# praveenpenumaka/splat-transform

Measured on AMD Instinct MI355X. Metric: Msplats/sec PLY->SOG (SH-3, 10 k-means iters), higher is better.
Workload: dtype f64+f32 (bit-exact JS semantics); fp16 MFMA (f32 accumulate) for the assign prefilter

## Files before the change

### splat-transform_amd/csrc/st_kmeans_nd.hip

```cpp
#include <cmath>
#include <cstring>
#include <utility>

#include "st_kmeans.h"

namespace st {
namespace {

using namespace km;

template <typename F, int... I>
__device__ inline void static_for_(F &f, std::integer_sequence<int, I...>) {
    (f(std::integral_constant<int, I>{}), ...);
}
template <int N, typename F>
__device__ inline void static_for(F &&f) {
    static_for_(f, std::make_integer_sequence<int, N>{});
}

typedef _Float16 f16x8 __attribute__((ext_vector_type(8)));
typedef float f32x16 __attribute__((ext_vector_type(16)));
typedef float f32x2 __attribute__((ext_vector_type(2)));

constexpr int PT = 4;
constexpr int NW = 4;
constexpr int WG = 64 * NW;
constexpr int CT_STAGE = 8;
enum { UPD_ALWAYS = 0, UPD_LANE = 1, UPD_WAVE = 2, UPD_BOTH = 3, UPD_DEFAULT = UPD_BOTH };
constexpr int CAND_CAP = 64;
constexpr int CAND_CAP2 = 2048;
constexpr int OVF_BATCH = 4096;
uint32_t sumnd_big() {
    const char *e = getenv("ST_SUMND_BIG");
    return e ? (uint32_t)std::max(1ul, strtoul(e, nullptr, 10)) : 16384u;
}

int sweep_update() {
    const char *e = getenv("ST_SWEEP_UPDATE");
    if (!e || !*e) return UPD_DEFAULT;
    if (!strcmp(e, "always")) return UPD_ALWAYS;
    if (!strcmp(e, "lane")) return UPD_LANE;
    if (!strcmp(e, "wave")) return UPD_WAVE;
    if (!strcmp(e, "both")) return UPD_BOTH;
    throw Error(ST_ERR_UNSUPPORTED, "ST_SWEEP_UPDATE: always, lane, wave or both");
}

__host__ __device__ inline int kp_of(int d) { return ((d + 3) + 15) / 16 * 16; }

__device__ inline uint16_t h_bits(float f) { return __builtin_bit_cast(uint16_t, (_Float16)f); }
__device__ inline float h_val(uint16_t b) { return (float)__builtin_bit_cast(_Float16, b); }

struct Bound {
    float r, a, b, ec, ep, rel;
};

Bound make_bound(int d, bool denorm) {
    const double u = std::ldexp(1.0, -11);
    const double e_abs = denorm ? std::ldexp(1.0, -25) : std::ldexp(1.0, -14);
    const double gam = (d + 3 + 3) * std::ldexp(1.0, -23);
    Bound B{};
    B.r = (float)(2 * 1.05);
    B.a = (float)(2.01 * gam * (1 + u) * (1 + u) * 1.05);
    B.b = (float)((1.01 * gam + std::ldexp(1.0, -22)) * 1.05);
    B.ec = (float)(2 * std::sqrt((double)d) * e_abs * (1 + u) * 1.05);
    B.ep = (float)((2 * d * e_abs * e_abs + 3 * e_abs) * 1.05 + 1e-30);
    B.rel = 1.0e-13f;
    return B;
}

__device__ inline float err_bound(const Bound &B, float pn, float dp, float cn, float dc) {
    const float pt = pn + dp, ct = cn + dc;
    return B.r * (pn * dc + dp * ct) + B.a * pt * ct + B.b * ct * ct + B.ec * (pt + ct) + B.ep;
}

constexpr int NTAB = 1024;
__device__ inline uint32_t norm_bucket(float x, float scale) {
    return (uint32_t)fminf(x * scale, (float)(NTAB - 1));
}
__global__ __launch_bounds__(NTAB) void k_norm_table(const float *__restrict__ cnorm, const float *__restrict__ cdn,
                                                     uint32_t rows, const uint32_t *__restrict__ cmax_bits,
                                                     float *__restrict__ tab) {
    __shared__ uint32_t m[NTAB];
    const uint32_t t = threadIdx.x;
    m[t] = 0u;
    __syncthreads();
    const float cm = __builtin_bit_cast(float, cmax_bits[0]);
    const float scale = cm > 0.f ? (float)NTAB / cm : 0.f;
    for (uint32_t r = t; r < rows; r += NTAB) {
        const uint32_t b = norm_bucket(cnorm[r], scale), v = __builtin_bit_cast(uint32_t, cdn[r]);
        if (v > __hip_atomic_load(&m[b], __ATOMIC_RELAXED, __HIP_MEMORY_SCOPE_WORKGROUP)) atomicMax(&m[b], v);
    }
    __syncthreads();
    for (uint32_t o = 1; o < (uint32_t)NTAB; o <<= 1) {
        const uint32_t v = t >= o ? m[t - o] : 0u;
        __syncthreads();
        m[t] = max(m[t], v);
        __syncthreads();
    }
    tab[t] = __builtin_bit_cast(float, m[t]);
}

__device__ inline float norm_reach(float pn, float t) {
    const float q = pn * pn + t;
    const float qe = q + 0x1p-19f * (pn * pn + __builtin_fabsf(t));
    return (pn + __builtin_sqrtf(fmaxf(0.f, qe))) * (1.0f + 0x1p-18f);
}

__device__ inline float wbound_r(const Bound &B, float pn, float dp, float cb, float dcb, float cm, float ntab_scale,
                                 const float *__restrict__ ntab, float m1u) {
    const float e0 = err_bound(B, pn, dp, cb, dcb);
    const float c1 = fminf(norm_reach(pn, m1u + e0 * 1.0001f), cb);
    const float eb = err_bound(B, pn, dp, c1, fminf(dcb, ntab[norm_bucket(c1, ntab_scale)]));
    const float sb = pn + c1, sm = pn + cm;
    const float t = m1u + eb * 1.0001f + B.rel * (sb * sb + sm * sm);
    const float cr = fminf(norm_reach(pn, t), cm);
    const float dcr = ntab[norm_bucket(cr, ntab_scale)];
    const float sr = pn + cr;
    return (eb + err_bound(B, pn, dp, cr, dcr) + B.rel * (sb * sb + sr * sr)) * 1.0001f;
}

__device__ inline float wbound_pair(const Bound &B, float pn, float dp, float ca, float dca, float cb, float dcb) {
    const float s = pn + fmaxf(ca, cb);
    return (err_bound(B, pn, dp, ca, dca) + err_bound(B, pn, dp, cb, dcb) + 2.0f * B.rel * s * s) * 1.0001f;
}

__global__ __launch_bounds__(256) void k_half_max(const float *__restrict__ cnorm, const float *__restrict__ cdn,
                                                  uint32_t nhalves, float *__restrict__ chalf,
                                                  float *__restrict__ chalf_d) {
    for (uint32_t h = blockIdx.x * blockDim.x + threadIdx.x; h < nhalves; h += gridDim.x * blockDim.x) {
        float m = 0.f, md = 0.f;
        for (int rr = 0; rr < 16; ++rr) {
            const uint32_t r = (h >> 1) * 32 + 4 * (h & 1) + (rr & 3) + 8 * (rr >> 2);
            m = fmaxf(m, cnorm[r]);
            md = fmaxf(md, cdn[r]);
        }
        chalf[h] = m;
        chalf_d[h] = md;
    }
}

__global__ void k_probe_denorm(float *out) {
    const int lane = threadIdx.x;
    f16x8 a = {}, b = {};
    if (lane == 0) {
        a[0] = __builtin_bit_cast(_Float16, (uint16_t)0x0010u);
        b[0] = (_Float16)1.0f;
    }
    f32x16 acc = {};
    acc = __builtin_amdgcn_mfma_f32_32x32x16_f16(a, b, acc, 0, 0, 0);
    if (lane == 0) out[0] = acc[0];
}

__global__ __launch_bounds__(256) void k_absmax(const float *const *cols, int d, uint64_t n, uint32_t *out) {
    const uint64_t stride = (uint64_t)gridDim.x * blockDim.x;
    float m = 0.f;
    for (uint64_t i = (uint64_t)blockIdx.x * blockDim.x + threadIdx.x; i < n; i += stride)
        for (int c = 0; c < d; ++c) m = fmaxf(m, __builtin_fabsf(cols[c][i]));
    for (int o = 32; o > 0; o >>= 1) m = fmaxf(m, __shfl_xor(m, o, 64));
    if ((threadIdx.x & 63) == 0) atomicMax(out, __builtin_bit_cast(uint32_t, m));
}

constexpr int PF_PTS = 128;
constexpr int PF_LDS_LD = PF_PTS + 1;
template <int DT>
__global__ __launch_bounds__(PF_PTS) void k_point_frags(const float *const *cols, int d_rt, uint64_t n, uint32_t ntiles,
                                                     int ks_rt, float sigma, uint4 *pfrag, float *pnorm, float *pdn,
                                                     float *aos) {
    __shared__ float x[(DT ? DT : 61) * PF_LDS_LD];
    const int d = DT ? DT : d_rt;
    const int ks = DT ? kp_of(DT) / 16 : ks_rt;
    const uint64_t p0 = (uint64_t)blockIdx.x * PF_PTS;
    const int j = threadIdx.x;
    const bool valid = p0 + j < n;
    const uint64_t pj = valid ? p0 + j : n - 1;
    if constexpr (DT > 0) {
        float v[DT];
#pragma unroll
        for (int u = 0; u < DT; ++u) v[u] = cols[u][pj];
#pragma unroll
        for (int u = 0; u < DT; ++u) x[u * PF_LDS_LD + j] = valid ? v[u] : 0.0f;
    } else {
        int k0 = 0;
        for (; k0 + 8 <= d; k0 += 8) {
            float v[8];
#pragma unroll
            for (int u = 0; u < 8; ++u) v[u] = cols[k0 + u][pj];
#pragma unroll
            for (int u = 0; u < 8; ++u) x[(k0 + u) * PF_LDS_LD + j] = valid ? v[u] : 0.0f;
        }
        for (; k0 < d; ++k0) x[k0 * PF_LDS_LD + j] = valid ? cols[k0][pj] : 0.0f;
    }
    __syncthreads();
    if (valid) {
        double nn = 0, dd = 0;
        for (int k = 0; k < d; ++k) {
            const float f = x[k * PF_LDS_LD + j] * sigma;
            const double v = (double)f, r = v - (double)h_val(h_bits(f));
            nn += v * v;
            dd += r * r;
        }
        pnorm[p0 + j] = (float)(__builtin_sqrt(nn) * (1.0 + 1e-6));
        pdn[p0 + j] = (float)(__builtin_sqrt(dd) * (1.0 + 1e-6));
    }
    const int ld = aos_ld(d), q4 = ld / 4;
    const uint32_t rows = (uint32_t)min((uint64_t)PF_PTS, n - min(n, p0));
    float4 *dst = reinterpret_cast<float4 *>(aos + p0 * ld);
    for (uint32_t f = j; f < rows * q4; f += PF_PTS) {
        const uint32_t r = f / q4, c = (f % q4) * 4;
        float4 v;
        v.x = c + 0 < (uint32_t)d ? x[(c + 0) * PF_LDS_LD + r] : 0.0f;
        v.y = c + 1 < (uint32_t)d ? x[(c + 1) * PF_LDS_LD + r] : 0.0f;
        v.z = c + 2 < (uint32_t)d ? x[(c + 2) * PF_LDS_LD + r] : 0.0f;
        v.w = c + 3 < (uint32_t)d ? x[(c + 3) * PF_LDS_LD + r] : 0.0f;
        dst[f] = v;
    }
    const uint32_t t0 = blockIdx.x * (PF_PTS / 32);
    const uint32_t tiles = min((uint32_t)(PF_PTS / 32), ntiles - t0);
    for (uint32_t f = j; f < tiles * ks * 64; f += PF_PTS) {
        const uint32_t t = f / (ks * 64), rem = f % (ks * 64);
        const int st = (int)(rem / 64), h = (int)((rem % 64) / 32), l = (int)(rem % 32);
        const uint32_t r = t * 32 + l;
        const bool pv = p0 + r < n;
        uint16_t e[8];
#pragma unroll
        for (int jj = 0; jj < 8; ++jj) {
            const int k = 16 * st + 8 * h + jj;
            uint16_t bits = 0;
            if (k < d) {
                if (pv) bits = h_bits(-2.0f * h_val(h_bits(x[k * PF_LDS_LD + r] * sigma)));
            } else if (k < d + 3) {
                bits = pv ? (uint16_t)0x3c00u : (uint16_t)0;
            }
            e[jj] = bits;
        }
        uint4 v;
        v.x = e[0] | ((uint32_t)e[1] << 16);
        v.y = e[2] | ((uint32_t)e[3] << 16);
        v.z = e[4] | ((uint32_t)e[5] << 16);
        v.w = e[6] | ((uint32_t)e[7] << 16);
        pfrag[(uint64_t)(t0 + t) * ks * 64 + rem] = v;
    }
}

constexpr int CF_W = 4;
__global__ __launch_bounds__(64 * CF_W) void k_centroid_frags(const float *cen, int d, int k, uint32_t ctiles, int ks,
                                                              float sigma, uint4 *cfrag, uint32_t *cmax_bits,
                                                              float *caos, float2 *cfix, float *cnorm, float *cdn) {
    __shared__ double pn[CF_W][64], pd[CF_W][64];
    const uint32_t total = ctiles * 32;
    const int ld = aos_ld(d);
    const int lane = threadIdx.x & 63;
    const int w = __builtin_amdgcn_readfirstlane(threadIdx.x >> 6);
    const int per = (ld / 2 + CF_W - 1) / CF_W * 2;
    const int c0 = w * per, c1 = min(ld, c0 + per);
    float mymax = 0.f, mydmax = 0.f;
    for (uint32_t rb = blockIdx.x; rb * 64 < total; rb += gridDim.x) {
        const uint32_t r = rb * 64 + lane;
        const bool live = r < total;
        const bool valid = live && r < (uint32_t)k;
        double nn = 0, dd = 0;
        if (valid) {
            const uint32_t row = r & 31, hh = (row >> 2) & 1, r16 = (row & 3) | ((row >> 3) << 2);
            for (int c = c0; c < c1; c += 2) {
                const float a = c < d ? cen[(uint64_t)c * k + r] : 0.0f;
                const float b = c + 1 < d ? cen[(uint64_t)(c + 1) * k + r] : 0.0f;
                caos[(uint64_t)r * ld + c] = a;
                caos[(uint64_t)r * ld + c + 1] = b;
                cfix[(((uint64_t)(r >> 5) * 2 + hh) * (ld / 2) + c / 2) * 16 + r16] = make_float2(a, b);
            }
            for (int c = c0; c < min(c1, d); ++c) {
                const float f = cen[(uint64_t)c * k + r] * sigma;
                const double x = (double)f, e = x - (double)h_val(h_bits(f));
                nn += x * x;
                dd += e * e;
            }
        }
        pn[w][lane] = nn;
        pd[w][lane] = dd;
        __syncthreads();
        nn = ((pn[0][lane] + pn[1][lane]) + pn[2][lane]) + pn[3][lane];
        dd = ((pd[0][lane] + pd[1][lane]) + pd[2][lane]) + pd[3][lane];
        __syncthreads();
        static_assert(CF_W == 4, "the fixed-order sum above");
        if (!live || w >= ks) continue;
        uint16_t n1, n2, n3;
        if (valid) {
            n1 = h_bits((float)nn);
            const double r1 = nn - (double)h_val(n1);
            n2 = h_bits((float)r1);
            const double r2 = r1 - (double)h_val(n2);
            n3 = h_bits((float)r2);
            if (w == 0) {
                const float nr = (float)(__builtin_sqrt(nn) * (1.0 + 1e-6));
                const float dr = (float)(__builtin_sqrt(dd) * (1.0 + 1e-6));
                mymax = fmaxf(mymax, nr);
                mydmax = fmaxf(mydmax, dr);
                cnorm[r] = nr;
                cdn[r] = dr;
            }
        } else {
            if (w == 0) {
                cnorm[r] = 0.0f;
                cdn[r] = 0.0f;
            }
            n1 = h_bits(60000.0f);
            n2 = n3 = 0;
        }
        const int s = w;
        const uint32_t t = r >> 5, row = r & 31;
        for (int h = 0; h < 2; ++h) {
            uint16_t e[8];
#pragma unroll
            for (int j = 0; j < 8; ++j) {
                const int kk = 16 * s + 8 * h + j;
                uint16_t bits = 0;
                if (kk < d) bits = valid ? h_bits(cen[(uint64_t)kk * k + r] * sigma) : (uint16_t)0;
                else if (kk == d) bits = n1;
                else if (kk == d + 1) bits = n2;
                else if (kk == d + 2) bits = n3;
                e[j] = bits;
            }
            uint4 v;
            v.x = e[0] | ((uint32_t)e[1] << 16);
            v.y = e[2] | ((uint32_t)e[3] << 16);
            v.z = e[4] | ((uint32_t)e[5] << 16);
            v.w = e[6] | ((uint32_t)e[7] << 16);
            cfrag[((uint64_t)t * ks + s) * 64 + h * 32 + row] = v;
        }
    }
    for (int o = 32; o > 0; o >>= 1) {
        mymax = fmaxf(mymax, __shfl_xor(mymax, o, 64));
        mydmax = fmaxf(mydmax, __shfl_xor(mydmax, o, 64));
    }
    if (lane == 0 && w == 0) {
        atomicMax(cmax_bits, __builtin_bit_cast(uint32_t, mymax));
        atomicMax(cmax_bits + 1, __builtin_bit_cast(uint32_t, mydmax));
    }
}

template <int KS, int MODE, int UPD = UPD_ALWAYS>
__global__ __launch_bounds__(WG) void k_sweep(const uint4 *__restrict__ pfrag, uint32_t ntiles, uint32_t npts,
                                               const uint4 *__restrict__ cfrag, uint32_t ctiles,
                                               const float *__restrict__ pnorm, const float *__restrict__ pdn,
                                               const uint32_t *__restrict__ cmax_bits, const float *__restrict__ chalf,
                                               const float *__restrict__ chalf_d, const float *__restrict__ ntab,
                                               const Bound bnd, uint32_t *__restrict__ labels,
                                               float *__restrict__ thr, uint32_t *__restrict__ amb, State *st,
                                               uint32_t *__restrict__ cand_cnt, uint32_t *__restrict__ cand,
                                               uint32_t cand_cap,
                                               uint32_t *__restrict__ pair_pts, uint2 *__restrict__ pair_codes,
                                               uint32_t *__restrict__ code_hist) {
    constexpr int STAGE_U4 = CT_STAGE * KS * 64;
    constexpr int PER_THREAD = (STAGE_U4 + WG - 1) / WG;
    static_assert(STAGE_U4 % 64 == 0, "a stage is whole wave-instructions");
    __shared__ uint4 lds[2][STAGE_U4];
    const int lane = threadIdx.x & 63, w = threadIdx.x >> 6, h = lane >> 5;
    const uint32_t tile0 = (blockIdx.x * NW + w) * PT;

    f16x8 b[PT][KS];
#pragma unroll
    for (int t = 0; t < PT; ++t) {
        const uint32_t tt = tile0 + t;
#pragma unroll
        for (int s = 0; s < KS; ++s) {
            uint4 q = (tt < ntiles) ? pfrag[((uint64_t)tt * KS + s) * 64 + lane] : make_uint4(0, 0, 0, 0);
            b[t][s] = __builtin_bit_cast(f16x8, q);
        }
    }
    float ninf;
    asm volatile("v_mov_b32 %0, 0xff800000" : "=v"(ninf));
    const uint32_t kbits = ctiles > 1 ? 32u - (uint32_t)__builtin_clz(ctiles - 1) : 0u;
    const uint32_t kmask = (1u << kbits) - 1u;
    float m1[PT], m2[PT], m3[PT], th[PT];
    float m3u[PT];
    const float gdk = __builtin_ldexpf(1.0f, (int)kbits - 21);
    auto guard_of = [&](float m) { return __builtin_fmaf(__builtin_fabsf(m), gdk, m) + 0x1p-126f; };
    bool full[PT];
    uint32_t kmask_v;
    asm volatile("v_mov_b32 %0, %1" : "=v"(kmask_v) : "s"(kmask));
#pragma unroll
    for (int t = 0; t < PT; ++t) {
        m1[t] = __builtin_inff();
        m2[t] = __builtin_inff();
        m3[t] = __builtin_inff();
        m3u[t] = __builtin_inff();
        th[t] = -__builtin_inff();
        full[t] = false;
        if (MODE == 1) {
            const uint32_t slot = (tile0 + t) * 32 + (lane & 31);
            if (slot < npts) th[t] = thr[slot];
        }
    }

    float mn = 0.f;
    auto slice = [&](const f32x16 &sc, int t, uint32_t ctile, auto qc) {
        constexpr int q = decltype(qc)::value;
        constexpr int r0 = q * 16 / KS, r1 = (q + 1) * 16 / KS;
        if (q == 0) mn = sc[0];
#pragma unroll
        for (int r = (q == 0 ? 1 : r0); r < r1; ++r) mn = fminf(mn, sc[r]);
        if (q == KS - 1) {
            if (MODE == 0) {
                auto update = [&] {
                    uint32_t kb;
                    asm("v_bfi_b32 %0, %1, %2, %3" : "=v"(kb) : "v"(kmask_v), "s"(ctile), "v"(mn));
                    const float key = __builtin_bit_cast(float, kb);
                    m3[t] = __builtin_amdgcn_fmed3f(m2[t], m3[t], key);
                    m2[t] = __builtin_amdgcn_fmed3f(m1[t], m2[t], key);
                    m1[t] = fminf(m1[t], key);
                };
                if (UPD == UPD_ALWAYS) {
                    update();
                } else if (UPD == UPD_WAVE) {
                    if (__ballot(mn < m3u[t]) != 0) {
                        update();
                        m3u[t] = guard_of(m3[t]);
                    }
                } else if (UPD == UPD_LANE) {
                    if (mn < m3u[t]) {
                        update();
                        m3u[t] = guard_of(m3[t]);
                    }
                } else {
                    const bool below = mn < m3u[t];
                    if (__ballot(below) != 0) {
                        asm volatile("");
                        if (below) {
                            update();
                            m3u[t] = guard_of(m3[t]);
                        }
                    }
                }
            } else if (mn <= th[t] && !full[t]) {
                const uint32_t slot = (tile0 + t) * 32 + (lane & 31);
#pragma unroll
                for (int r = 0; r < 16; ++r) {
                    if (sc[r] <= th[t] && !full[t]) {
                        const uint32_t ci = ctile * 32 + 4 * h + (r & 3) + 8 * (r >> 2);
                        const uint32_t pos = atomicAdd(&cand_cnt[slot], 1u);
                        if (pos < cand_cap) cand[(uint64_t)slot * cand_cap + pos] = ci;
                        else full[t] = true;
                    }
                }
            }
        }
    };

    const uint32_t nstages = ctiles / CT_STAGE;
    const uint32_t sg_begin = MODE == 1 ? (uint32_t)((uint64_t)blockIdx.y * nstages / gridDim.y) : 0u;
    const uint32_t sg_end = MODE == 1 ? (uint32_t)((uint64_t)(blockIdx.y + 1) * nstages / gridDim.y) : nstages;
    const uint32_t wbase = __builtin_amdgcn_readfirstlane(w) * 64;
    auto stage_in = [&](int buf, uint32_t sg_) {
        const uint4 *src = cfrag + (uint64_t)sg_ * STAGE_U4 + threadIdx.x;
#pragma unroll
        for (int q = 0; q < PER_THREAD; ++q)
            if (STAGE_U4 % WG == 0 || wbase + q * WG < (uint32_t)STAGE_U4)
                __builtin_amdgcn_global_load_lds(src + q * WG,
                                                 (__attribute__((address_space(3))) void *)&lds[buf][wbase + q * WG],
                                                 16, 0, 0);
    };
    stage_in(0, sg_begin);
    asm volatile("s_waitcnt vmcnt(0)" ::: "memory");
    __syncthreads();
    static_assert(PT == 4, "the score-buffer rotation assumes 4 point tiles per wave");
    f32x16 buf[PT];
#pragma unroll
    for (int t = 0; t < PT; ++t)
#pragma unroll
        for (int r = 0; r < 16; ++r) buf[t][r] = 0x1p+120f;
    uint32_t tile_prev = 0;
    for (uint32_t sg = sg_begin; sg < sg_end; ++sg) {
        const int cur = (sg - sg_begin) & 1;
        if (sg + 1 < sg_end) stage_in(cur ^ 1, sg + 1);
        f16x8 a0[KS], a1[KS];
#pragma unroll
        for (int s = 0; s < KS; ++s) a0[s] = __builtin_bit_cast(f16x8, lds[cur][s * 64 + lane]);
        auto tile_step = [&](uint32_t ct, f16x8 (&a)[KS], f16x8 (&an)[KS]) {
            const uint32_t tile_cur = sg * CT_STAGE + ct;
            const uint32_t ctn = (ct + 1 < (uint32_t)CT_STAGE) ? ct + 1 : ct;
#pragma unroll
            for (int s = 0; s < KS; ++s) an[s] = __builtin_bit_cast(f16x8, lds[cur][(ctn * KS + s) * 64 + lane]);
            static_for<PT>([&](auto tc_) {
                constexpr int t = decltype(tc_)::value;
                constexpr int td = (t + 1) % PT;
                const uint32_t tile_d = (td > t) ? tile_prev : tile_cur;
                f32x16 acc = {};
                static_for<KS>([&](auto sc_) {
                    constexpr int s = decltype(sc_)::value;
                    acc = __builtin_amdgcn_mfma_f32_32x32x16_f16(a[s], b[t][s], acc, 0, 0, 0);
                    slice(buf[td], td, tile_d, sc_);
                    __builtin_amdgcn_sched_barrier(0);
                });
                buf[t] = acc;
            });
            tile_prev = tile_cur;
        };
        static_assert(CT_STAGE % 2 == 0, "ping-pong over pairs of centroid tiles");
#pragma unroll 1
        for (uint32_t ct = 0; ct < (uint32_t)CT_STAGE; ct += 2) {
            tile_step(ct, a0, a1);
            tile_step(ct + 1, a1, a0);
        }
        if (sg + 1 < sg_end) {
            asm volatile("s_waitcnt vmcnt(0)" ::: "memory");
            __syncthreads();
        }
    }
    static_for<PT - 1>([&](auto tc_) {
        constexpr int td = decltype(tc_)::value + 1;
        static_for<KS>([&](auto sc_) { slice(buf[td], td, tile_prev, sc_); });
    });
    if (MODE == 1) return;

    const float cm = __builtin_bit_cast(float, cmax_bits[0]);
    const float ntab_scale = cm > 0.f ? (float)NTAB / cm : 0.f;
#pragma unroll
    for (int t = 0; t < PT; ++t) {
        const float a1 = m1[t], a2 = m2[t], a3 = m3[t];
        const float b1 = __shfl_xor(a1, 32, 64), b2 = __shfl_xor(a2, 32, 64), b3 = __shfl_xor(a3, 32, 64);
        const uint32_t ca1 = (__builtin_bit_cast(uint32_t, a1) & kmask) * 2u + (uint32_t)h;
        const uint32_t ca2 = (__builtin_bit_cast(uint32_t, a2) & kmask) * 2u + (uint32_t)h;
        const uint32_t cb1 = __shfl_xor(ca1, 32, 64), cb2 = __shfl_xor(ca2, 32, 64);
        const float nm1 = fminf(a1, b1);
        const float nm2 = fminf(fmaxf(a1, b1), fminf(a2, b2));
        const float nm3 = fminf(fminf(a3, b3), fminf(fmaxf(a2, b1), fmaxf(a1, b2)));
        const uint32_t code1 = (a1 <= b1) ? ca1 : cb1;
        const uint32_t code2 = (a1 <= b1) ? ((a2 <= b1) ? ca2 : cb1) : ((b2 < a1) ? cb2 : ca1);
        const uint32_t p = (tile0 + t) * 32 + (lane & 31);
        bool is_amb = false, is_pair = false;
        if (h == 0 && p < npts) {
            const float kr = __builtin_ldexpf(1.0f, (int)kbits - 23) * 1.01f + 0x1p-20f, ka = 0x1p-126f;
            const float e1 = __builtin_fabsf(nm1) * kr + ka;
            const float pn = pnorm[p], dp = pdn[p];
            const float W = wbound_r(bnd, pn, dp, chalf[code1], chalf_d[code1], cm, ntab_scale, ntab, nm1 + e1);
            if (nm2 > nm1 + W + e1 + (__builtin_fabsf(nm2) * kr + ka)) {
                labels[p] = code1;
                if (code_hist) atomicAdd(&code_hist[code1], 1u);
            } else if (nm3 > nm1 + W + e1 + (__builtin_fabsf(nm3) * kr + ka)) {
                const float W2 = wbound_pair(bnd, pn, dp, chalf[code1], chalf_d[code1], chalf[code2], chalf_d[code2]);
                if (nm2 > nm1 + W2 + e1 + (__builtin_fabsf(nm2) * kr + ka)) {
                    labels[p] = code1;
                    if (code_hist) atomicAdd(&code_hist[code1], 1u);
                } else {
                    is_pair = true;
                    labels[p] = 0xfffffffeu;
                }
            } else {
                is_amb = true;
                labels[p] = 0xffffffffu;
                thr[p] = nm1 + e1 + W;
            }
        }
        const uint64_t pmask = __ballot(is_pair);
        if (pmask) {
            uint32_t base = 0;
            const int leader = __builtin_ctzll(pmask);
            if (lane == leader) base = atomicAdd(&st->pairs, (uint32_t)__popcll(pmask));
            base = __shfl(base, leader, 64);
            if (is_pair) {
                const uint32_t i = base + __popcll(pmask & ((1ull << lane) - 1));
                pair_pts[i] = p;
                pair_codes[i] = make_uint2(code1, code2);
            }
        }
        const uint64_t mask = __ballot(is_amb);
        if (mask) {
            uint32_t base = 0;
            const int leader = __builtin_ctzll(mask);
            if (lane == leader) base = atomicAdd(&st->amb, (uint32_t)__popcll(mask));
            base = __shfl(base, leader, 64);
            if (is_amb) amb[base + __popcll(mask & ((1ull << lane) - 1))] = p;
        }
    }
}

__global__ __launch_bounds__(256) void k_gather_amb(const uint4 *__restrict__ pfrag, const uint32_t *__restrict__ amb,
                                                    const float *__restrict__ thr_p, uint32_t namb, int ks,
                                                    uint4 *__restrict__ afrag, float *__restrict__ thr_slot,
                                                    uint32_t *__restrict__ cand_cnt) {
    const uint32_t total = (namb + 31) / 32 * 32;
    for (uint32_t a = blockIdx.x * blockDim.x + threadIdx.x; a < total; a += gridDim.x * blockDim.x) {
        const bool valid = a < namb;
        const uint32_t p = valid ? amb[a] : 0u;
        const uint32_t pt = p >> 5, pc = p & 31, at = a >> 5, ac = a & 31;
        for (int s = 0; s < ks; ++s)
            for (int h = 0; h < 2; ++h)
                afrag[((uint64_t)at * ks + s) * 64 + h * 32 + ac] =
                    valid ? pfrag[((uint64_t)pt * ks + s) * 64 + h * 32 + pc] : make_uint4(0, 0, 0, 0);
        thr_slot[a] = valid ? thr_p[p] : -__builtin_inff();
        cand_cnt[a] = 0;
    }
}

__device__ inline double ref_dist(const float *__restrict__ crow, const float *__restrict__ prow, int ld) {
    const float4 *c4 = reinterpret_cast<const float4 *>(crow);
    const float4 *p4 = reinterpret_cast<const float4 *>(prow);
    double l = 0;
    for (int q = 0; q < ld / 4; ++q) {
        const float4 a = c4[q], b = p4[q];
        double v = (double)a.x - (double)b.x;
        l += v * v;
        v = (double)a.y - (double)b.y;
        l += v * v;
        v = (double)a.z - (double)b.z;
        l += v * v;
        v = (double)a.w - (double)b.w;
        l += v * v;
    }
    return l;
}

__device__ inline uint32_t code_row(uint32_t code, int rr) {
    return (code >> 1) * 32 + 4 * (code & 1) + (rr & 3) + 8 * (rr >> 2);
}

struct FixOut {
    uint32_t label;
    bool tie;
};
template <int G>
__device__ inline FixOut fix_decide(float s, bool valid, uint32_t c, int d, const float *__restrict__ caos,
                                    const float *__restrict__ prow, uint64_t p, int r, uint32_t *__restrict__ labels,
                                    uint32_t *__restrict__ ties, State *st);

template <int CTRL>
__device__ inline uint32_t dpp_u(uint32_t x) {
    return (uint32_t)__builtin_amdgcn_update_dpp(0, (int)x, CTRL, 0xf, 0xf, false);
}
template <int CTRL>
__device__ inline float dpp_f(float x) {
    return __builtin_bit_cast(float, dpp_u<CTRL>(__builtin_bit_cast(uint32_t, x)));
}
__device__ inline float row16_min(float v) {
    v = fminf(v, dpp_f<0xB1>(v));
    v = fminf(v, dpp_f<0x4E>(v));
    v = fminf(v, dpp_f<0x124>(v));
    return fminf(v, dpp_f<0x128>(v));
}
__device__ inline uint32_t row16_umin(uint32_t v) {
    v = min(v, dpp_u<0xB1>(v));
    v = min(v, dpp_u<0x4E>(v));
    v = min(v, dpp_u<0x124>(v));
    return min(v, dpp_u<0x128>(v));
}
__device__ inline uint32_t row16_sum(uint32_t v) {
    v += dpp_u<0xB1>(v);
    v += dpp_u<0x4E>(v);
    v += dpp_u<0x124>(v);
    return v + dpp_u<0x128>(v);
}

template <int G>
__device__ inline void fix_group(const float *__restrict__ aos, int d, const float2 *__restrict__ cfix,
                                 const float *__restrict__ caos, int k, uint64_t p, int r, uint32_t code,
                                 uint32_t *__restrict__ labels, uint32_t *__restrict__ ties, State *st) {
    const int ld = aos_ld(d);
    const int rr = r & 15;
    const uint32_t c = code_row(code, rr);
    const bool valid = c < (uint32_t)k;
    const float *prow = aos + p * ld;
    float s = 0.f;
    if (valid) {
        const float4 *p4 = reinterpret_cast<const float4 *>(prow);
// ... 1024 lines not shown
                                                     const uint32_t *__restrict__ soff,
                                                     const uint32_t *__restrict__ nlist, double *__restrict__ psum,
                                                     double *__restrict__ pabs, int *__restrict__ pemin,
                                                     uint32_t *__restrict__ nzl, uint32_t *__restrict__ nzc) {
    __shared__ double ls[4][64], la[4][64];
    __shared__ int le[4][64];
    const int lane = threadIdx.x & 63, w = threadIdx.x >> 6;
    const int ld = aos_ld(d);
    const uint32_t nl = *nlist, total = soff[nl];
    for (uint32_t sl = blockIdx.x; sl < total; sl += gridDim.x) {
        uint32_t lo = 0, hi = nl;
        while (hi - lo > 1) {
            const uint32_t mid = (lo + hi) >> 1;
            if (soff[mid] <= sl) lo = mid;
            else hi = mid;
        }
        const uint32_t cl = list[lo];
        const uint32_t s0 = start[cl] + (sl - soff[lo]) * SB_SLICE;
        const uint32_t s1 = min(start[cl + 1], s0 + SB_SLICE);
        const uint32_t per = (s1 - s0 + 3) / 4;
        const uint32_t a = s0 + min(s1 - s0, w * per), b = s0 + min(s1 - s0, (w + 1) * per);
        double sum = 0, sabs = 0;
        int emin = 0x7fffffff;
        uint32_t *nz = nzl + ((uint64_t)sl * 4 + w) * SB_WAVE;
        uint32_t cnt = 0;
        auto take = [&](T x, uint32_t mem) {
            sum += (double)x;
            sabs += __builtin_fabs((double)x);
            if (x != 0) emin = min(emin, ulp_exp(x));
            if (__ballot(x != 0)) {
                if (lane == 0) nz[cnt] = mem;
                ++cnt;
            }
        };
        if (lane < d) {
            constexpr int U = 32;
            uint32_t j = a;
            for (; j + U <= b; j += U) {
                T v[U];
#pragma unroll
                for (int u = 0; u < U; ++u) v[u] = aos[(uint64_t)members[j + u] * ld + lane];
#pragma unroll
                for (int u = 0; u < U; ++u) take(v[u], members[j + u]);
            }
            for (; j < b; ++j) take(aos[(uint64_t)members[j] * ld + lane], members[j]);
            if (lane == 0) nzc[(uint64_t)sl * 4 + w] = cnt;
        }
        ls[w][lane] = sum;
        la[w][lane] = sabs;
        le[w][lane] = emin;
        __syncthreads();
        if (w == 0 && lane < d) {
            psum[(uint64_t)sl * 64 + lane] = ((ls[0][lane] + ls[1][lane]) + ls[2][lane]) + ls[3][lane];
            pabs[(uint64_t)sl * 64 + lane] = ((la[0][lane] + la[1][lane]) + la[2][lane]) + la[3][lane];
            pemin[(uint64_t)sl * 64 + lane] = min(min(le[0][lane], le[1][lane]), min(le[2][lane], le[3][lane]));
        }
        __syncthreads();
    }
}

template <typename T>
__global__ __launch_bounds__(64) void k_big_final(const T *__restrict__ aos, int d,
                                                  const uint32_t *__restrict__ members,
                                                  const uint32_t *__restrict__ start, int k,
                                                  const uint32_t *__restrict__ list, const uint32_t *__restrict__ soff,
                                                  const uint32_t *__restrict__ nlist, const double *__restrict__ psum,
                                                  const double *__restrict__ pabs, const int *__restrict__ pemin,
                                                  const uint32_t *__restrict__ nzl, const uint32_t *__restrict__ nzc,
                                                  float *__restrict__ cen) {
    const int lane = threadIdx.x;
    const int ld = aos_ld(d);
    const uint32_t nl = *nlist;
    for (uint32_t i = blockIdx.x; i < nl; i += gridDim.x) {
        if (lane >= d) continue;
        const uint32_t cl = list[i], s0 = start[cl], s1 = start[cl + 1], m = s1 - s0;
        double S = 0, A = 0;
        int E = 0x7fffffff;
        for (uint32_t sl = soff[i]; sl < soff[i + 1]; ++sl) {
            S += psum[(uint64_t)sl * 64 + lane];
            A += pabs[(uint64_t)sl * 64 + lane];
            E = min(E, pemin[(uint64_t)sl * 64 + lane]);
        }
        if (!sum_is_exact(A, E)) {
            S = 0;
            constexpr int U = 32;
            for (uint64_t part = (uint64_t)soff[i] * 4; part < (uint64_t)soff[i + 1] * 4; ++part) {
                const uint32_t *mem = nzl + part * SB_WAVE;
                const uint32_t c = nzc[part];
                uint32_t j = 0;
                for (; j + U <= c; j += U) {
                    T v[U];
#pragma unroll
                    for (int u = 0; u < U; ++u) v[u] = aos[(uint64_t)mem[j + u] * ld + lane];
#pragma unroll
                    for (int u = 0; u < U; ++u) S += (double)v[u];
                }
                for (; j < c; ++j) S += (double)aos[(uint64_t)mem[j] * ld + lane];
            }
        }
        (void)members;
        (void)s0;
        cen[(uint64_t)lane * k + cl] = (float)(S / (double)m);
    }
}

__global__ __launch_bounds__(256) void k_aos64(const double *const *cols, int d, uint64_t n, double *__restrict__ aos) {
    const int ld = aos_ld(d);
    for (uint64_t f = (uint64_t)blockIdx.x * blockDim.x + threadIdx.x; f < n * ld; f += (uint64_t)gridDim.x * blockDim.x) {
        const uint64_t r = f / ld;
        const int a = (int)(f % ld);
        aos[f] = a < d ? cols[a][r] : 0.0;
    }
}

template <typename T>
void big_sums(st_ctx *c, const T *aos, int d, uint64_t n, int k, const uint32_t *members, const uint32_t *start,
              float *cen, uint32_t cap, uint32_t *list, uint32_t *nlist) {
    const uint64_t slices = n / SB_SLICE + cap;
    auto *soff = wsT<uint32_t>(c, "kn.bsoff", (size_t)cap + 1);
    auto *psum = wsT<double>(c, "kn.bsum", slices * 64);
    auto *pabs = wsT<double>(c, "kn.babs", slices * 64);
    auto *pemin = wsT<int>(c, "kn.bemin", slices * 64);
    auto *nzl = wsT<uint32_t>(c, "kn.bnzl", slices * 4 * SB_WAVE);
    auto *nzc = wsT<uint32_t>(c, "kn.bnzc", slices * 4);
    hipLaunchKernelGGL(k_big_prefix, dim3(1), dim3(64), 0, c->stream, start, cap, list, soff, nlist);
    hipLaunchKernelGGL(k_big_partial<T>, dim3(grid_for(slices, 1, 2048)), dim3(256), 0, c->stream, aos, d, members,
                       start, list, soff, nlist, psum, pabs, pemin, nzl, nzc);
    hipLaunchKernelGGL(k_big_final<T>, dim3(std::min<unsigned>(cap, 1024u)), dim3(64), 0, c->stream, aos, d, members,
                       start, k, list, soff, nlist, psum, pabs, pemin, nzl, nzc, cen);
    ST_LAUNCH_CHECK();
}

template <typename T>
void launch_sums(st_ctx *c, const T *aos, int d, uint64_t n, int k, const uint32_t *members, const uint32_t *start,
                 float *cen, const uint32_t *only = nullptr, const uint32_t *nonly = nullptr, uint32_t rows = 0) {
    const uint32_t big = sumnd_big();
    const uint32_t cap = (uint32_t)(n / ((uint64_t)big + 1) + 1);
    auto *list = wsT<uint32_t>(c, "kn.blist", cap);
    auto *nlist = wsT<uint32_t>(c, "kn.bn", 1);
    ST_HIP(hipMemsetAsync(nlist, 0, 4, c->stream));
    hipLaunchKernelGGL(k_sumnd<T>, dim3(((only ? rows : k) + 3) / 4), dim3(256), 0, c->stream, aos, d, members, start,
                       k, cen, big, cap, list, nlist, only, nonly);
    if (n > big) big_sums(c, aos, d, n, k, members, start, cen, cap, list, nlist);
    ST_LAUNCH_CHECK();
}

template <int KS>
struct Sweep {
    static void main(st_ctx *c, const uint4 *pfrag, uint32_t ntiles, uint32_t n, const uint4 *cfrag, uint32_t ctiles,
                     const float *pnorm, const float *pdn, const uint32_t *cmax, const float *chalf,
                     const float *chalf_d, const float *ntab, const Bound &bnd,
                     uint32_t *labels, float *thr, uint32_t *amb, State *st, uint32_t *pair_pts, uint2 *pair_codes,
                     uint32_t *code_hist) {
        const uint32_t per_block = NW * PT;
        const dim3 grid((ntiles + per_block - 1) / per_block);
        KTimer kt(c, "kn.sweep");
        auto launch = [&](auto kernel) {
            hipLaunchKernelGGL(kernel, grid, dim3(WG), 0, c->stream, pfrag, ntiles, n, cfrag, ctiles, pnorm, pdn,
                               cmax, chalf, chalf_d, ntab, bnd, labels, thr, amb, st, (uint32_t *)nullptr,
                               (uint32_t *)nullptr, 0u, pair_pts, pair_codes, code_hist);
        };
        switch (sweep_update()) {
            case UPD_LANE: launch(k_sweep<KS, 0, UPD_LANE>); break;
            case UPD_WAVE: launch(k_sweep<KS, 0, UPD_WAVE>); break;
            case UPD_BOTH: launch(k_sweep<KS, 0, UPD_BOTH>); break;
            default: launch(k_sweep<KS, 0, UPD_ALWAYS>); break;
        }
        ST_LAUNCH_CHECK();
    }
    static void collect(st_ctx *c, const uint4 *afrag, uint32_t atiles, uint32_t namb, const uint4 *cfrag,
                        uint32_t ctiles, const Bound &bnd, float *thr_slot, uint32_t *cand_cnt, uint32_t *cand,
                        uint32_t cap, hipStream_t s) {
        const uint32_t per_block = NW * PT;
        const uint32_t blocks = (atiles + per_block - 1) / per_block;
        const uint32_t split = std::max(1u, std::min(ctiles / CT_STAGE, (2048u + blocks - 1) / blocks));
        const dim3 grid(blocks, split);
        KTimer kt(c, "kn.collect", s);
        hipLaunchKernelGGL((k_sweep<KS, 1>), grid, dim3(WG), 0, s, afrag, atiles, namb, cfrag, ctiles,
                           (const float *)nullptr, (const float *)nullptr, (const uint32_t *)nullptr,
                           (const float *)nullptr, (const float *)nullptr, (const float *)nullptr, bnd,
                           (uint32_t *)nullptr, thr_slot,
                           (uint32_t *)nullptr, (State *)nullptr, cand_cnt, cand, cap, (uint32_t *)nullptr,
                           (uint2 *)nullptr, (uint32_t *)nullptr);
        ST_LAUNCH_CHECK();
    }
};

bool probe_denorm(st_ctx *c) {
    static thread_local std::map<int, bool> cache;
    auto it = cache.find(c->device);
    if (it != cache.end()) return it->second;
    auto *d = wsT<float>(c, "kn.probe", 1);
    hipLaunchKernelGGL(k_probe_denorm, dim3(1), dim3(64), 0, c->stream, d);
    ST_LAUNCH_CHECK();
    float v = 0;
    ST_HIP(hipMemcpyAsync(&v, d, 4, hipMemcpyDeviceToHost, c->stream));
    ST_HIP(hipStreamSynchronize(c->stream));
    const bool keep = (v == std::ldexp(1.0f, -20));
    cache[c->device] = keep;
    return keep;
}

}

#define ST_KS_DISPATCH(KSV, CALL) \
    switch (KSV) {                \
        case 1: { constexpr int KS = 1; CALL; } break; \
        case 2: { constexpr int KS = 2; CALL; } break; \
        case 3: { constexpr int KS = 3; CALL; } break; \
        case 4: { constexpr int KS = 4; CALL; } break; \
        default: throw Error(ST_ERR_UNSUPPORTED, "kmeans: dimension too large for the MFMA assign (D <= 61)"); \
    }
#define ST_LD_DISPATCH(LDV, ...)                               \
    switch (LDV) {                                             \
        case 48: { constexpr int LD = 48; __VA_ARGS__; } break; \
        case 24: { constexpr int LD = 24; __VA_ARGS__; } break; \
        default: { constexpr int LD = 12; __VA_ARGS__; } break; \
    }
#define ST_DT_DISPATCH(DV, ...)                                \
    switch (DV) {                                              \
        case 45: { constexpr int DT = 45; __VA_ARGS__; } break; \
        case 24: { constexpr int DT = 24; __VA_ARGS__; } break; \
        case 9: { constexpr int DT = 9; __VA_ARGS__; } break;   \
        default: { constexpr int DT = 0; __VA_ARGS__; } break;  \
    }
static bool palette_ld(int ld) { return ld == 48 || ld == 24 || ld == 12; }

void nd_prepare(st_ctx *c, const float *const *dcols, int d, uint64_t n) {
    ST_REQUIRE(d <= 61, ST_ERR_UNSUPPORTED, "kmeans: D > 61 not supported by the MFMA assign");
    const int ks = kp_of(d) / 16;
    const uint32_t ntiles = (uint32_t)((n + 31) / 32);
    auto *pfrag = wsT<uint4>(c, "kn.pfrag", (size_t)ntiles * ks * 64);
    auto *pnorm = wsT<float>(c, "kn.pnorm", n);
    auto *pdn = wsT<float>(c, "kn.pdn", n);
    auto *aos = wsT<float>(c, "kn.aos", n * (size_t)aos_ld(d));
    auto *scal = wsT<uint32_t>(c, "kn.scal", 4);
    ST_HIP(hipMemsetAsync(scal, 0, 16, c->stream));
    float amax = c->km_absmax;
    c->km_absmax = -1.0f;
    if (amax < 0.0f) {
        hipLaunchKernelGGL(k_absmax, dim3(grid_for(n, 256, 2048)), dim3(256), 0, c->stream, dcols, d, n, scal);
        ST_LAUNCH_CHECK();
        uint32_t amax_bits = 0;
        ST_HIP(hipMemcpyAsync(&amax_bits, scal, 4, hipMemcpyDeviceToHost, c->stream));
        ST_HIP(hipStreamSynchronize(c->stream));
        amax = __builtin_bit_cast(float, amax_bits);
    }
    float sigma = 1.0f;
    if (amax > 0) sigma = std::ldexp(1.0f, -std::ilogb(amax));
    const dim3 gpf((unsigned)(((uint64_t)ntiles * 32 + PF_PTS - 1) / PF_PTS));
    ST_DT_DISPATCH(d, hipLaunchKernelGGL(k_point_frags<DT>, gpf, dim3(PF_PTS), 0, c->stream, dcols, d, n, ntiles, ks,
                                         sigma, pfrag, pnorm, pdn, aos));
    ST_LAUNCH_CHECK();
    c->kn_sigma = sigma;
    c->kn_n = n;
    c->kn_d = d;
    mark(c, "kn.prep");
}

namespace {
__global__ __launch_bounds__(256) void k_rows_aos(const float *__restrict__ cen, int d, int k, float *__restrict__ caos) {
    const int ld = aos_ld(d);
    for (uint64_t f = (uint64_t)blockIdx.x * blockDim.x + threadIdx.x; f < (uint64_t)k * ld;
         f += (uint64_t)gridDim.x * blockDim.x) {
        const uint32_t r = (uint32_t)(f / ld), a = (uint32_t)(f % ld);
        caos[f] = a < (uint32_t)d ? cen[(uint64_t)a * k + r] : 0.0f;
    }
}


struct Assign {
    st_ctx *c;
    int d;
    uint64_t n;
    int k;
    uint32_t *labels;
    State *dstate;
    int ld = aos_ld(d), ks = kp_of(d) / 16;
    uint32_t ntiles = (uint32_t)((n + 31) / 32);
    uint32_t ctiles = (uint32_t)(((k + 31) / 32 + CT_STAGE - 1) / CT_STAGE * CT_STAGE);
    uint32_t ncodes = ctiles * 2;
    Bound bnd = make_bound(d, probe_denorm(c));
    const uint4 *pfrag = wsT<uint4>(c, "kn.pfrag", (size_t)ntiles * ks * 64);
    const float *pnorm = wsT<float>(c, "kn.pnorm", n);
    const float *pdn = wsT<float>(c, "kn.pdn", n);
    const float *aos = wsT<float>(c, "kn.aos", n * (size_t)ld);
    uint32_t *scal = wsT<uint32_t>(c, "kn.scal", 4);
    uint4 *cfrag = wsT<uint4>(c, "kn.cfrag", (size_t)ctiles * ks * 64);
    float *thr = wsT<float>(c, "kn.thr", n);
    uint32_t *amb = wsT<uint32_t>(c, "kn.amb", n);
    uint32_t *ties = wsT<uint32_t>(c, "kn.ties", n);
    float *caos = wsT<float>(c, "kn.caos", (size_t)k * ld);
    float2 *cfix = wsT<float2>(c, "kn.cfix", (size_t)ctiles * 32 * (ld / 2));
    float *cnorm = wsT<float>(c, "kn.cnorm", (size_t)ctiles * 32);
    float *chalf = wsT<float>(c, "kn.chalf", (size_t)ctiles * 2);
    float *cdn = wsT<float>(c, "kn.cdn", (size_t)ctiles * 32);
    float *chalf_d = wsT<float>(c, "kn.chalfd", (size_t)ctiles * 2);
    float *ntab = wsT<float>(c, "kn.ntab", NTAB);
    uint32_t *pair_pts = wsT<uint32_t>(c, "kn.pairpts", n);
    uint2 *pair_codes = wsT<uint2>(c, "kn.paircodes", n);
};

void prepare_centroids(st_ctx *c, const Assign &a, const float *cen) {
    ST_HIP(hipMemsetAsync(a.scal + 1, 0, 8, c->stream));
    ST_REQUIRE(a.ks <= CF_W, ST_ERR_INTERNAL, "kmeans: more fragments per row than centroid waves");
    hipLaunchKernelGGL(k_centroid_frags, dim3(grid_for((uint64_t)a.ctiles * 32, 64, 4096)), dim3(64 * CF_W), 0,
                       c->stream, cen, a.d, a.k, a.ctiles, a.ks, c->kn_sigma, a.cfrag, a.scal + 1, a.caos, a.cfix,
                       a.cnorm, a.cdn);
    hipLaunchKernelGGL(k_half_max, dim3(grid_for((uint64_t)a.ctiles * 2, 256, 1024)), dim3(256), 0, c->stream, a.cnorm,
                       a.cdn, a.ctiles * 2, a.chalf, a.chalf_d);
    hipLaunchKernelGGL(k_norm_table, dim3(1), dim3(NTAB), 0, c->stream, a.cnorm, a.cdn, a.ctiles * 32, a.scal + 1,
                       a.ntab);
    ST_LAUNCH_CHECK();
}

struct FusedWs {
    st_ctx *c;
    uint64_t n;
    int ld;
    uint32_t ncodes;
    uint64_t slices = ncodes + n / FA_SL + 1;
    uint32_t *soff = wsT<uint32_t>(c, "kn.fasoff", (size_t)ncodes + 1);
    double *psum = wsT<double>(c, "kn.fasum", slices * 16 * ld);
    double *pabs = wsT<double>(c, "kn.faabs", slices * 16 * ld);
    int *pemin = wsT<int>(c, "kn.faemin", slices * 16 * ld);
    uint32_t *pcnt = wsT<uint32_t>(c, "kn.facnt", slices * 16);
// ... 417 lines not shown
```

Measured before the change: 21.18.

## Widen k-means sweep to 8 point tiles per wave with 3-buffer score rotation

After: 21.29 (median of 6 runs). Within noise of the previous version (+0.5%).

```diff
diff --git a/splat-transform_amd/csrc/st_kmeans_nd.hip b/splat-transform_amd/csrc/st_kmeans_nd.hip
--- a/splat-transform_amd/csrc/st_kmeans_nd.hip
+++ b/splat-transform_amd/csrc/st_kmeans_nd.hip
@@ -22,7 +22,10 @@
 typedef float f32x16 __attribute__((ext_vector_type(16)));
 typedef float f32x2 __attribute__((ext_vector_type(2)));
 
-constexpr int PT = 4;
+constexpr int PT_NARROW = 4;
+constexpr int PT_WIDE = 8;
+constexpr int NBUF_WIDE = 3;
+constexpr int PT_DEFAULT = PT_WIDE;
 constexpr int NW = 4;
 constexpr int WG = 64 * NW;
 constexpr int CT_STAGE = 8;
@@ -43,6 +46,14 @@
     if (!strcmp(e, "wave")) return UPD_WAVE;
     if (!strcmp(e, "both")) return UPD_BOTH;
     throw Error(ST_ERR_UNSUPPORTED, "ST_SWEEP_UPDATE: always, lane, wave or both");
+}
+
+int sweep_pt() {
+    const char *e = getenv("ST_SWEEP_PT");
+    if (!e || !*e) return PT_DEFAULT;
+    if (!strcmp(e, "4")) return PT_NARROW;
+    if (!strcmp(e, "8")) return PT_WIDE;
+    throw Error(ST_ERR_UNSUPPORTED, "ST_SWEEP_PT: 4 or 8");
 }
 
 __host__ __device__ inline int kp_of(int d) { return ((d + 3) + 15) / 16 * 16; }
@@ -338,8 +349,23 @@
     }
 }
 
-template <int KS, int MODE, int UPD = UPD_ALWAYS>
-__global__ __launch_bounds__(WG) void k_sweep(const uint4 *__restrict__ pfrag, uint32_t ntiles, uint32_t npts,
+template <int PT, int NBUF>
+struct Rotation {
+    static constexpr bool even = PT % NBUF == 0;
+    static_assert(NBUF >= 3 && NBUF - 1 <= PT, "one buffer written, one settling, one draining");
+    static_assert(even || (NBUF == 3 && PT % 3 == 2), "NBUF divides PT, or NBUF = 3 and PT = 3 m + 2");
+    static constexpr int pending = even ? PT - (NBUF - 1) : PT - 1;
+    static constexpr int count(int t) { return even ? 1 : t == PT - 1 ? 2 : t == 1 ? 0 : 1; }
+    static constexpr int tile(int t, int j) { return even ? (t + PT - (NBUF - 1)) % PT : t == 0 ? PT - 1 : t - 2 + j; }
+    static constexpr bool prev(int t) { return even ? t < NBUF - 1 : t == 0; }
+    static constexpr int gap(int t, int i, int ks) {
+        return even || (t >= 2 && t < PT - 1) ? i : t == PT - 1 ? i / 2 : (i + 1 < ks ? i + 1 : ks - 1);
+    }
+};
+
+template <int KS, int MODE, int UPD = UPD_ALWAYS, int PT = PT_NARROW, int NBUF = PT_NARROW>
+__global__ __launch_bounds__(WG) __attribute__((amdgpu_waves_per_eu(PT > 4 ? 2 : 1, PT > 4 ? 2 : 8)))
+void k_sweep(const uint4 *__restrict__ pfrag, uint32_t ntiles, uint32_t npts,
                                                const uint4 *__restrict__ cfrag, uint32_t ctiles,
                                                const float *__restrict__ pnorm, const float *__restrict__ pdn,
                                                const uint32_t *__restrict__ cmax_bits, const float *__restrict__ chalf,
@@ -462,10 +488,10 @@
     stage_in(0, sg_begin);
     asm volatile("s_waitcnt vmcnt(0)" ::: "memory");
     __syncthreads();
-    static_assert(PT == 4, "the score-buffer rotation assumes 4 point tiles per wave");
-    f32x16 buf[PT];
-#pragma unroll
-    for (int t = 0; t < PT; ++t)
+    using Rot = Rotation<PT, NBUF>;
+    f32x16 buf[NBUF];
+#pragma unroll
+    for (int t = 0; t < NBUF; ++t)
 #pragma unroll
         for (int r = 0; r < 16; ++r) buf[t][r] = 0x1p+120f;
     uint32_t tile_prev = 0;
@@ -482,16 +508,21 @@
             for (int s = 0; s < KS; ++s) an[s] = __builtin_bit_cast(f16x8, lds[cur][(ctn * KS + s) * 64 + lane]);
             static_for<PT>([&](auto tc_) {
                 constexpr int t = decltype(tc_)::value;
-                constexpr int td = (t + 1) % PT;
-                const uint32_t tile_d = (td > t) ? tile_prev : tile_cur;
+                const uint32_t tile_d = Rot::prev(t) ? tile_prev : tile_cur;
                 f32x16 acc = {};
                 static_for<KS>([&](auto sc_) {
                     constexpr int s = decltype(sc_)::value;
                     acc = __builtin_amdgcn_mfma_f32_32x32x16_f16(a[s], b[t][s], acc, 0, 0, 0);
-                    slice(buf[td], td, tile_d, sc_);
+                    static_for<2 * KS>([&](auto ic_) {
+                        constexpr int i = decltype(ic_)::value;
+                        if constexpr (i < Rot::count(t) * KS && Rot::gap(t, i, KS) == s) {
+                            constexpr int td = Rot::tile(t, i / KS);
+                            slice(buf[td % NBUF], td, tile_d, std::integral_constant<int, i % KS>{});
+                        }
+                    });
                     __builtin_amdgcn_sched_barrier(0);
                 });
-                buf[t] = acc;
+                buf[t % NBUF] = acc;
             });
             tile_prev = tile_cur;
         };
@@ -506,9 +537,9 @@
             __syncthreads();
         }
     }
-    static_for<PT - 1>([&](auto tc_) {
-        constexpr int td = decltype(tc_)::value + 1;
-        static_for<KS>([&](auto sc_) { slice(buf[td], td, tile_prev, sc_); });
+    static_for<PT - Rot::pending>([&](auto tc_) {
+        constexpr int td = decltype(tc_)::value + Rot::pending;
+        static_for<KS>([&](auto sc_) { slice(buf[td % NBUF], td, tile_prev, sc_); });
     });
     if (MODE == 1) return;
 
@@ -1839,6 +1870,22 @@
                      const float *chalf_d, const float *ntab, const Bound &bnd,
                      uint32_t *labels, float *thr, uint32_t *amb, State *st, uint32_t *pair_pts, uint2 *pair_codes,
                      uint32_t *code_hist) {
+        const int upd = sweep_update(), pt = sweep_pt();
+        if constexpr (KS <= 3) {
+            if (pt == PT_WIDE)
+                return main_as<PT_WIDE, NBUF_WIDE>(c, upd, pfrag, ntiles, n, cfrag, ctiles, pnorm, pdn, cmax, chalf,
+                                                   chalf_d, ntab, bnd, labels, thr, amb, st, pair_pts, pair_codes,
+                                                   code_hist);
+        }
+        main_as<PT_NARROW, PT_NARROW>(c, upd, pfrag, ntiles, n, cfrag, ctiles, pnorm, pdn, cmax, chalf, chalf_d, ntab,
+                                      bnd, labels, thr, amb, st, pair_pts, pair_codes, code_hist);
+    }
+    template <int PT, int NBUF>
+    static void main_as(st_ctx *c, int upd, const uint4 *pfrag, uint32_t ntiles, uint32_t n, const uint4 *cfrag,
+                        uint32_t ctiles, const float *pnorm, const float *pdn, const uint32_t *cmax,
+                        const float *chalf, const float *chalf_d, const float *ntab, const Bound &bnd,
+                        uint32_t *labels, float *thr, uint32_t *amb, State *st, uint32_t *pair_pts,
+                        uint2 *pair_codes, uint32_t *code_hist) {
         const uint32_t per_block = NW * PT;
         const dim3 grid((ntiles + per_block - 1) / per_block);
         KTimer kt(c, "kn.sweep");
@@ -1847,18 +1894,18 @@
                                cmax, chalf, chalf_d, ntab, bnd, labels, thr, amb, st, (uint32_t *)nullptr,
                                (uint32_t *)nullptr, 0u, pair_pts, pair_codes, code_hist);
         };
-        switch (sweep_update()) {
-            case UPD_LANE: launch(k_sweep<KS, 0, UPD_LANE>); break;
-            case UPD_WAVE: launch(k_sweep<KS, 0, UPD_WAVE>); break;
-            case UPD_BOTH: launch(k_sweep<KS, 0, UPD_BOTH>); break;
-            default: launch(k_sweep<KS, 0, UPD_ALWAYS>); break;
+        switch (upd) {
+            case UPD_LANE: launch(k_sweep<KS, 0, UPD_LANE, PT, NBUF>); break;
+            case UPD_WAVE: launch(k_sweep<KS, 0, UPD_WAVE, PT, NBUF>); break;
+            case UPD_BOTH: launch(k_sweep<KS, 0, UPD_BOTH, PT, NBUF>); break;
+            default: launch(k_sweep<KS, 0, UPD_ALWAYS, PT, NBUF>); break;
         }
         ST_LAUNCH_CHECK();
     }
     static void collect(st_ctx *c, const uint4 *afrag, uint32_t atiles, uint32_t namb, const uint4 *cfrag,
                         uint32_t ctiles, const Bound &bnd, float *thr_slot, uint32_t *cand_cnt, uint32_t *cand,
                         uint32_t cap, hipStream_t s) {
-        const uint32_t per_block = NW * PT;
+        const uint32_t per_block = NW * PT_NARROW;
         const uint32_t blocks = (atiles + per_block - 1) / per_block;
         const uint32_t split = std::max(1u, std::min(ctiles / CT_STAGE, (2048u + blocks - 1) / blocks));
         const dim3 grid(blocks, split);
```
